# TobiasWooldridge/WaveCap-SDR

Measured on AMD Instinct MI355X. Metric: input IQ MS/s x channels demodulated (1024-channel polyphase filterbank), higher is better.
Workload: dtype f32

## Files before the change

### wavecap-sdr_amd/csrc/pfb.hip

```cpp
#include "pfb_internal.h"
#include "wh_common.h"
#include <cmath>
#include <cstdint>
#include <cstdlib>
#include <memory>
#include <vector>

using namespace wh;

namespace {

constexpr int FM = 1024;
constexpr int FHOP = 512;
constexpr int FT = 9;
constexpr int GH = 4;
constexpr int LDS1_K1 = 272;

template <int FMT>
__device__ __forceinline__ float2 ld_iq(const void *p, long long i) {
    if (FMT == 1) {
        short2 v = reinterpret_cast<const short2 *>(p)[i];
        return make_float2((float)v.x * (1.0f / 32768.0f), (float)v.y * (1.0f / 32768.0f));
    }
    return reinterpret_cast<const float2 *>(p)[i];
}
template <int FMT>
__device__ __forceinline__ float2 ld_iq_raw(const void *p, long long i) {
    if (FMT == 1) {
        short2 v = reinterpret_cast<const short2 *>(p)[i];
        return make_float2((float)v.x, (float)v.y);
    }
    return reinterpret_cast<const float2 *>(p)[i];
}
__device__ __forceinline__ float2 ld_iq_rt(const void *p, int fmt, long long i) {
    return fmt == 1 ? ld_iq<1>(p, i) : ld_iq<0>(p, i);
}

struct PfbFastArgs {
    const void *x;
    float2 *out;
    const float *arms;
    const float2 *tw1024;
    long long first_hop;
    long long n_groups;
    int groups_per_wg;
    int n_wg;
    int alt_dir;
    int map_chunk;
    long long max_block;
    double *stats_ws;
#ifdef WH_DIAG
    int ablate;
#endif
};

typedef float p2f __attribute__((ext_vector_type(2)));
#define P_SW(a) __builtin_shufflevector(a, a, 1, 0)
#define P_XX(a) __builtin_shufflevector(a, a, 0, 0)
#define P_YY(a) __builtin_shufflevector(a, a, 1, 1)
#define P_FMA(a, b, c) __builtin_elementwise_fma(a, b, c)
#define P_PMI(x, d) P_FMA(P_SW(d), (p2f{1.f, -1.f}), x)
#define P_MMI(x, d) P_FMA(P_SW(d), (p2f{-1.f, 1.f}), x)
__device__ __forceinline__ p2f pcmul(p2f a, p2f w) {
    const p2f t = P_XX(a) * w;
    const p2f s = P_YY(a) * p2f{-1.f, 1.f};
    return P_FMA(s, P_SW(w), t);
}
__device__ __forceinline__ p2f pcmulc(p2f a, float wx, float wy) {
    return P_FMA(P_YY(a), (p2f{-wy, wx}), (P_XX(a) * p2f{wx, wy}));
}
__device__ __forceinline__ void pfft4(p2f &a0, p2f &a1, p2f &a2, p2f &a3) {
    const p2f s02 = a0 + a2, d02 = a0 - a2, s13 = a1 + a3, d13 = a1 - a3;
    a0 = s02 + s13;
    a2 = s02 - s13;
    a1 = P_PMI(d02, d13);
    a3 = P_MMI(d02, d13);
}
__device__ __forceinline__ void pfft16(p2f (&v)[16]) {
    constexpr float C1 = 0.92387953251128673848f, S1 = 0.38268343236508978178f, R2 = 0.70710678118654752440f;
#pragma unroll
    for (int na = 0; na < 4; ++na) pfft4(v[na], v[na + 4], v[na + 8], v[na + 12]);
    v[5] = pcmulc(v[5], C1, -S1);
    v[9] = P_PMI(v[9], v[9]) * p2f{R2, R2};
    v[13] = pcmulc(v[13], S1, -C1);
    v[6] = P_PMI(v[6], v[6]) * p2f{R2, R2};
    v[10] = P_SW(v[10]) * p2f{1.f, -1.f};
    v[14] = P_MMI(v[14], v[14]) * p2f{-R2, -R2};
    v[7] = pcmulc(v[7], S1, -C1);
    v[11] = P_MMI(v[11], v[11]) * p2f{-R2, -R2};
    v[15] = pcmulc(v[15], -C1, S1);
#pragma unroll
    for (int kb = 0; kb < 4; ++kb) pfft4(v[4 * kb], v[4 * kb + 1], v[4 * kb + 2], v[4 * kb + 3]);
#pragma unroll
    for (int a = 0; a < 4; ++a)
#pragma unroll
        for (int b = a + 1; b < 4; ++b) {
            const p2f tmp = v[a + 4 * b];
            v[a + 4 * b] = v[b + 4 * a];
            v[b + 4 * a] = tmp;
        }
}

template <int FMT, bool GLDS, bool STATS, bool W3>
struct Pfb1024Lds {
    static constexpr int LDS_HOP = W3 ? 1088 : 1152;
    static constexpr int PRE_BYTES = GLDS ? GH * FHOP * (FMT == 1 ? 4 : 8) : 0;
    static constexpr bool PRE_SINGLE = W3 && FMT == 0;
    static constexpr int WORDS = GH * LDS_HOP + 256 + (PRE_SINGLE ? 1 : 2) * PRE_BYTES / 8;
};

template <int FMT, bool GLDS, bool STATS, bool W3, int DIR>
__device__ __forceinline__ void pfb1024_body(const PfbFastArgs &a, float2 *lds, long long g0, long long g1) {
    constexpr bool ST8 = W3;
    constexpr int LDS2_ROW = W3 ? 17 : 18;
    constexpr int LDS_HOP = Pfb1024Lds<FMT, GLDS, STATS, W3>::LDS_HOP;
    constexpr int PRE_BYTES = Pfb1024Lds<FMT, GLDS, STATS, W3>::PRE_BYTES;
    constexpr bool PRE_SINGLE = Pfb1024Lds<FMT, GLDS, STATS, W3>::PRE_SINGLE;
    float2 *tw256 = lds + GH * LDS_HOP;
    unsigned char *pre0 = reinterpret_cast<unsigned char *>(lds + GH * LDS_HOP + 256);
    constexpr int NEW0 = DIR > 0 ? 9 : 0;

    const int t = threadIdx.x;
    const int lane = t & 63;
    const int wave = t >> 6;

    const float2 tw256_t = a.tw1024[(4 * (t & 15) * (t >> 4)) & 1023];
    float2 tw1 = a.tw1024[t], tw2 = a.tw1024[(2 * t) & 1023], tw3 = a.tw1024[(3 * t) & 1023];
    long long h = a.first_hop + (DIR > 0 ? g0 : g1 - 1) * GH;
    float2 wA[9 + GH], wB[9 + GH];
    const long long xp = (h - 8) * FHOP + t;
#pragma unroll
    for (int i = 0; i < 9 + GH; ++i) {
        wA[i] = ld_iq_raw<FMT>(a.x, xp + i * FHOP);
        wB[i] = ld_iq_raw<FMT>(a.x, xp + i * FHOP + 256);
    }
    typedef float v2f __attribute__((ext_vector_type(2)));
    v2f tpr[(4 * FT) / 2];
#pragma unroll
    for (int e = 0; e < 4 * FT; e += 2) {
        const int q0 = e / FT, j0 = e - q0 * FT, q1 = (e + 1) / FT, j1 = (e + 1) - q1 * FT;
        constexpr float TS = FMT == 1 ? 1.0f / 32768.0f : 1.0f;
        tpr[e / 2] = v2f{a.arms[(t + 256 * q0) * FT + j0] * TS, a.arms[(t + 256 * q1) * FT + j1] * TS};
    }
    tw256[t] = tw256_t;
    __syncthreads();
    const p2f tw1p = {tw1.x, tw1.y}, tw2p = {tw2.x, tw2.y}, tw3p = {tw3.x, tw3.y};
    const p2f tw1r = {-tw1.y, tw1.x}, tw2r = {-tw2.y, tw2.x}, tw3r = {-tw3.y, tw3.x};

    StAcc sacc[STATS ? 4 : 1];
    if (STATS) {
#pragma unroll
        for (int q = 0; q < 4; ++q) stacc_init(sacc[q]);
    }

    constexpr int NJ = GLDS ? PRE_BYTES / 16 / 256 : 0;
    auto dma_copy = [&](unsigned char *dst, long long blk) {
#ifdef WH_DIAG
        if (a.ablate & 2) blk = 9 + (blk & 15);
#endif
        const unsigned char *src = reinterpret_cast<const unsigned char *>(a.x) + (size_t)blk * FHOP * (FMT == 1 ? 4 : 8);
#pragma unroll
        for (int j = 0; j < NJ; ++j) {
            const unsigned char *gp = src + (size_t)(j * 256 + t) * 16;
            unsigned base = (unsigned)(uintptr_t)dst + (unsigned)(j * 256 + wave * 64) * 16;
            base = __builtin_amdgcn_readfirstlane(base);
            unsigned save;
            asm volatile("s_mov_b32 %0, m0\n\t"
                         "s_mov_b32 m0, %1\n\t"
                         "global_load_lds_dwordx4 %2, off\n\t"
                         "s_mov_b32 m0, %0"
                         : "=&s"(save) : "s"(base), "v"(gp) : "memory");
        }
    };
    __builtin_amdgcn_s_waitcnt(0x0F70);
    const long long ng = g1 - g0;
    for (long long it = 0; it < ng; ++it, h += DIR * GH) {
        const bool more = it + 1 < ng;
        unsigned char *pre = pre0 + ((!PRE_SINGLE && (it & 1)) ? PRE_BYTES : 0);
#pragma unroll
        for (int e = 0; e < (4 * FT) / 2; ++e) asm volatile("" : "+v"(tpr[e]));
#define WH_TAP(q, j) ((((q) * FT + (j)) & 1) ? __builtin_shufflevector(tpr[((q) * FT + (j)) >> 1], tpr[((q) * FT + (j)) >> 1], 1, 1) \
                                             : __builtin_shufflevector(tpr[((q) * FT + (j)) >> 1], tpr[((q) * FT + (j)) >> 1], 0, 0))
#define WH_V2(f) (v2f{(f).x, (f).y})
#pragma unroll
        for (int i = 0; i < GH; ++i) {
            v2f p0 = {0.f, 0.f}, p1 = p0, p2 = p0, p3 = p0;
#pragma unroll
            for (int j = 0; j < FT; ++j) {
                p0 = __builtin_elementwise_fma(WH_V2(wA[i + 8 - j]), WH_TAP(0, j), p0);
                p1 = __builtin_elementwise_fma(WH_V2(wB[i + 8 - j]), WH_TAP(1, j), p1);
                p2 = __builtin_elementwise_fma(WH_V2(wA[i + 9 - j]), WH_TAP(2, j), p2);
                p3 = __builtin_elementwise_fma(WH_V2(wB[i + 9 - j]), WH_TAP(3, j), p3);
            }
            pfft4(p0, p1, p2, p3);
            p2f *L = reinterpret_cast<p2f *>(lds + i * LDS_HOP);
            L[t] = p0;
            L[LDS1_K1 + t] = P_FMA(P_YY(p1), tw1r, (P_XX(p1) * tw1p));
            L[2 * LDS1_K1 + t] = P_FMA(P_YY(p2), tw2r, (P_XX(p2) * tw2p));
            L[3 * LDS1_K1 + t] = P_FMA(P_YY(p3), tw3r, (P_XX(p3) * tw3p));
        }
        if (DIR > 0) {
#pragma unroll
            for (int i = 0; i < 9; ++i) {
                wA[i] = wA[i + GH];
                wB[i] = wB[i + GH];
            }
        } else {
#pragma unroll
            for (int i = 8; i >= 0; --i) {
                wA[i + GH] = wA[i];
                wB[i + GH] = wB[i];
            }
        }
        const long long nblk = DIR > 0 ? h + GH + 1 : h - GH - 8;
        auto issue_dma = [&]() {
            if (more) dma_copy(pre, nblk);
        };
        if (GLDS) {
            if (!PRE_SINGLE) issue_dma();
        } else {
#pragma unroll
            for (int i = 0; i < GH; ++i) {
                long long blk = nblk + i;
                blk = blk > a.max_block ? a.max_block : (DIR < 0 && blk < 0 ? 0 : blk);
                wA[NEW0 + i] = ld_iq_raw<FMT>(a.x, blk * FHOP + t);
                wB[NEW0 + i] = ld_iq_raw<FMT>(a.x, blk * FHOP + t + 256);
            }
        }
        __syncthreads();
        if (GLDS && PRE_SINGLE) issue_dma();
        {
            p2f *L = reinterpret_cast<p2f *>(lds + wave * LDS_HOP);
            const int k1 = lane >> 4, n3 = lane & 15;
            p2f v[16];
            {
                const p2f *src = L + k1 * LDS1_K1 + n3;
#pragma unroll
                for (int n2 = 0; n2 < 16; ++n2) v[n2] = src[n2 * 16];
            }
            pfft16(v);
            __builtin_amdgcn_wave_barrier();
            p2f *dst = L + k1 * LDS2_ROW + n3;
            const p2f *twp = reinterpret_cast<const p2f *>(tw256);
            dst[0] = v[0];
#pragma unroll
            for (int k2 = 1; k2 < 16; ++k2) dst[k2 * 4 * LDS2_ROW] = pcmul(v[k2], twp[k2 * 16 + n3]);
        }
        __builtin_amdgcn_wave_barrier();
        {
            float2 *L = lds + wave * LDS_HOP;
            p2f v[16];
            if (W3) {
                const p2f *src = reinterpret_cast<const p2f *>(L) + lane * LDS2_ROW;
#pragma unroll
                for (int j = 0; j < 16; ++j) v[j] = src[j];
            } else {
                typedef float f4 __attribute__((ext_vector_type(4)));
                const unsigned addr = static_cast<unsigned>(reinterpret_cast<uintptr_t>(L + lane * LDS2_ROW));
                f4 r0, r1, r2, r3, r4, r5, r6, r7;
                asm volatile("ds_read_b128 %0, %8\n\t"
                             "ds_read_b128 %1, %8 offset:16\n\t"
                             "ds_read_b128 %2, %8 offset:32\n\t"
                             "ds_read_b128 %3, %8 offset:48\n\t"
                             "ds_read_b128 %4, %8 offset:64\n\t"
                             "ds_read_b128 %5, %8 offset:80\n\t"
                             "ds_read_b128 %6, %8 offset:96\n\t"
                             "ds_read_b128 %7, %8 offset:112\n\t"
                             "s_waitcnt lgkmcnt(0)"
                             : "=&v"(r0), "=&v"(r1), "=&v"(r2), "=&v"(r3), "=&v"(r4), "=&v"(r5), "=&v"(r6), "=&v"(r7)
                             : "v"(addr)
                             : "memory");
                __builtin_amdgcn_sched_barrier(0);
                v[0] = p2f{r0.x, r0.y};   v[1] = p2f{r0.z, r0.w};
                v[2] = p2f{r1.x, r1.y};   v[3] = p2f{r1.z, r1.w};
                v[4] = p2f{r2.x, r2.y};   v[5] = p2f{r2.z, r2.w};
                v[6] = p2f{r3.x, r3.y};   v[7] = p2f{r3.z, r3.w};
                v[8] = p2f{r4.x, r4.y};   v[9] = p2f{r4.z, r4.w};
                v[10] = p2f{r5.x, r5.y};  v[11] = p2f{r5.z, r5.w};
                v[12] = p2f{r6.x, r6.y};  v[13] = p2f{r6.z, r6.w};
                v[14] = p2f{r7.x, r7.y};  v[15] = p2f{r7.z, r7.w};
            }
            pfft16(v);
            float2 vf[16];
#pragma unroll
            for (int j = 0; j < 16; ++j) vf[j] = make_float2(v[j].x, v[j].y);
            if (STATS) {
                float *pwv = reinterpret_cast<float *>(L);
#pragma unroll
                for (int j = 0; j < 16; ++j) pwv[lane + 64 * j] = stat_power(vf[j].x, vf[j].y);
            } else if (ST8) {
                float2 *o = a.out + (h + wave) * FM + lane;
#pragma unroll
                for (int j = 0; j < 16; ++j)
#ifdef WH_DIAG
                    if (!(a.ablate & 1) || vf[j].x == 1.2345e30f)
#endif
                    o[64 * j] = vf[j];
            } else {
                const bool even = (lane & 1) == 0;
                float4 *o4 = reinterpret_cast<float4 *>(a.out + (h + wave) * FM + (lane & ~1) + (even ? 0 : 512));
#pragma unroll
                for (int j = 0; j < 8; ++j) {
                    float2 snd = even ? vf[j + 8] : vf[j];
                    float2 rcv;
                    rcv.x = __shfl_xor(snd.x, 1);
                    rcv.y = __shfl_xor(snd.y, 1);
                    float2 lo = even ? vf[j] : rcv;
                    float2 hi = even ? rcv : vf[j + 8];
#ifdef WH_DIAG
                    if (!(a.ablate & 1) || lo.x == 1.2345e30f)
#endif
                    o4[32 * j] = make_float4(lo.x, lo.y, hi.x, hi.y);
                }
            }
        }
        if (STATS) {
            __syncthreads();
#pragma unroll
            for (int q = 0; q < 4; ++q)
#pragma unroll
                for (int w = 0; w < GH; ++w)
                    stacc_add(sacc[q], reinterpret_cast<const float *>(lds + w * LDS_HOP)[t + 256 * q]);
            if (((it + 1) & 3) == 0) {
#pragma unroll
                for (int q = 0; q < 4; ++q) stacc_fold(sacc[q]);
            }
        }
        if (GLDS) {
#ifdef WH_DIAG
            if (a.ablate) asm volatile("s_waitcnt vmcnt(0)" ::: "memory");
            else
#endif
            if (STATS) asm volatile("s_waitcnt vmcnt(0)" ::: "memory");
            else if (ST8) asm volatile("s_waitcnt vmcnt(16)" ::: "memory");
            else asm volatile("s_waitcnt vmcnt(8)" ::: "memory");
        }
        __syncthreads();
        if (GLDS && more) {
#pragma unroll
            for (int i = 0; i < GH; ++i) {
                if (FMT == 1) {
                    const short2 *p16 = reinterpret_cast<const short2 *>(pre);
                    const short2 va = p16[i * FHOP + t], vb = p16[i * FHOP + t + 256];
                    wA[NEW0 + i] = make_float2((float)va.x, (float)va.y);
                    wB[NEW0 + i] = make_float2((float)vb.x, (float)vb.y);
                } else {
                    const float2 *p32 = reinterpret_cast<const float2 *>(pre);
                    wA[NEW0 + i] = p32[i * FHOP + t];
                    wB[NEW0 + i] = p32[i * FHOP + t + 256];
                }
            }
        }
    }
    if (STATS) {
        double *row = a.stats_ws + (size_t)blockIdx.x * 4 * FM;
#pragma unroll
        for (int q = 0; q < 4; ++q) {
            stacc_fold(sacc[q]);
            const int c = t + 256 * q;
            row[c] = sacc[q].s;
            row[FM + c] = sacc[q].s2;
            row[2 * FM + c] = (double)sacc[q].mn;
            row[3 * FM + c] = (double)sacc[q].mx;
        }
    }
}

template <int FMT, bool GLDS = false, bool STATS = false, bool W3 = false>
__global__ __launch_bounds__(256) __attribute__((amdgpu_waves_per_eu(W3 ? 3 : 2))) void pfb1024_kernel(PfbFastArgs a) {
    __shared__ __attribute__((aligned(16))) float2 lds[Pfb1024Lds<FMT, GLDS, STATS, W3>::WORDS];
    int b = blockIdx.x;
    int nwg = a.n_wg;
    int per = nwg >> 3;
    int run;
    if (a.map_chunk > 0) {
        const int i = b >> 3, ch = i / a.map_chunk;
        run = (ch * 8 + (b & 7)) * a.map_chunk + (i - ch * a.map_chunk);
    } else if (a.map_chunk == -2) {
        run = (nwg & 7) == 0 ? (b & 7) * per + (b >> 3) : b;
    } else {
        run = b;
    }

    long long g0 = (long long)run * a.groups_per_wg;
    long long g1 = g0 + a.groups_per_wg;
    if (g1 > a.n_groups) g1 = a.n_groups;
    if (g0 >= g1) {
        if (STATS) {
            double *row = a.stats_ws + (size_t)blockIdx.x * 4 * FM;
            for (int c = threadIdx.x; c < FM; c += 256) { row[c] = 0.0; row[FM + c] = 0.0; row[2 * FM + c] = INFINITY; row[3 * FM + c] = 0.0; }
        }
        return;
    }

    if (W3 && !STATS && a.alt_dir && (run & 1)) pfb1024_body<FMT, GLDS, STATS, W3, -1>(a, lds, g0, g1);
    else pfb1024_body<FMT, GLDS, STATS, W3, 1>(a, lds, g0, g1);
}

struct PfbGenArgs {
    const void *x;
    int fmt;
    const float2 *hist;
    float2 *out;
    const float *arms;
    const float2 *tw;
    int M, T, log2M;
    int n_radix;
    int radix[16];
    long long hop0;
    long long n_hops;
    long long hop0b;
    long long n_hops_b;
    long long row_b;
};

__device__ __forceinline__ float2 gen_block(const PfbGenArgs &a, long long g, int k) {
    if (g >= 0) return ld_iq_rt(a.x, a.fmt, g * (a.M / 2) + k);
    int col = (int)(-g - 1);
    if (col >= a.T) return make_float2(0.f, 0.f);
    return a.hist[(size_t)k * a.T + col];
}

__global__ __launch_bounds__(256) void pfb_generic_kernel(PfbGenArgs a) {
    extern __shared__ __attribute__((aligned(16))) float2 sm[];
    const long long h = (long long)blockIdx.x < a.n_hops ? a.hop0 + blockIdx.x
                                                          : a.hop0b + ((long long)blockIdx.x - a.n_hops);
    const int M = a.M, T = a.T;
    for (int k = threadIdx.x; k < M; k += blockDim.x) {
        float re = 0.f, im = 0.f;
        for (int j = 0; j < T; ++j) {
            float2 c = gen_block(a, h - j, k);
            float w = a.arms[(size_t)k * T + j];
            re = fmaf(c.x, w, re);
            im = fmaf(c.y, w, im);
        }
        sm[k] = make_float2(re, im);
    }
    __syncthreads();
    const bool in_b = (long long)blockIdx.x >= a.n_hops;
    float2 *o = a.out + (size_t)((in_b && a.row_b >= 0) ? a.row_b + (h - a.hop0b) : h) * M;
    if (a.n_radix > 0) {
        float2 *src = sm, *dst = sm + M;
        int n = M, s = 1;
        for (int st = 0; st < a.n_radix; ++st) {
            const int r = a.radix[st];
            const int m = n / r;
            for (int i = threadIdx.x; i < M / r; i += blockDim.x) {
                const int pp = i / s, q = i - pp * s;
                const float2 *x = src + q + s * pp;
                float2 *y = dst + q + s * r * pp;
                const int sm_ = s * m;
                const int tws = pp * s;
                if (r == 2) {
                    float2 c0 = x[0], c1 = x[sm_];
                    y[0] = cadd(c0, c1);
                    y[s] = cmul(csub(c0, c1), a.tw[tws]);
                } else if (r == 4) {
                    float2 v0 = x[0], v1 = x[sm_], v2 = x[2 * sm_], v3 = x[3 * sm_];
                    fft4(v0, v1, v2, v3);
                    y[0] = v0;
                    y[s] = cmul(v1, a.tw[tws]);
                    y[2 * s] = cmul(v2, a.tw[2 * tws]);
                    y[3 * s] = cmul(v3, a.tw[3 * tws]);
                } else if (r == 3) {
                    const float C = -0.5f, S = -0.86602540378443864676f;
                    float2 v0 = x[0], v1 = x[sm_], v2 = x[2 * sm_];
                    float2 t1 = cadd(v1, v2), t2 = csub(v1, v2);
                    float2 u = make_float2(fmaf(C, t1.x, v0.x), fmaf(C, t1.y, v0.y));
                    float2 w = make_float2(-S * t2.y, S * t2.x);
                    y[0] = cadd(v0, t1);
                    y[s] = cmul(cadd(u, w), a.tw[tws]);
                    y[2 * s] = cmul(csub(u, w), a.tw[2 * tws]);
                } else {
                    const float C1 = 0.30901699437494742410f, S1 = 0.95105651629515357212f;
                    const float C2 = -0.80901699437494742410f, S2 = 0.58778525229247312917f;
                    float2 v0 = x[0], v1 = x[sm_], v2 = x[2 * sm_], v3 = x[3 * sm_], v4 = x[4 * sm_];
                    float2 a1 = cadd(v1, v4), b1 = csub(v1, v4), a2 = cadd(v2, v3), b2 = csub(v2, v3);
                    float2 r1 = make_float2(v0.x + C1 * a1.x + C2 * a2.x, v0.y + C1 * a1.y + C2 * a2.y);
                    float2 r2 = make_float2(v0.x + C2 * a1.x + C1 * a2.x, v0.y + C2 * a1.y + C1 * a2.y);
                    float2 i1 = make_float2(S1 * b1.y + S2 * b2.y, -(S1 * b1.x + S2 * b2.x));
                    float2 i2 = make_float2(S2 * b1.y - S1 * b2.y, -(S2 * b1.x - S1 * b2.x));
                    y[0] = make_float2(v0.x + a1.x + a2.x, v0.y + a1.y + a2.y);
                    y[s] = cmul(cadd(r1, i1), a.tw[tws]);
                    y[2 * s] = cmul(cadd(r2, i2), a.tw[2 * tws]);
                    y[3 * s] = cmul(csub(r2, i2), a.tw[3 * tws]);
                    y[4 * s] = cmul(csub(r1, i1), a.tw[4 * tws]);
                }
            }
            __syncthreads();
            float2 *tmp = src; src = dst; dst = tmp;
            n = m; s *= r;
        }
        for (int k = threadIdx.x; k < M; k += blockDim.x) o[k] = src[k];
    } else if (a.log2M > 0) {
        float2 *src = sm, *dst = sm + M;
        const int half = M >> 1;
        int n = M, s = 1;
        for (int st = 0; st < a.log2M; ++st) {
            const int m = n >> 1;
            for (int i = threadIdx.x; i < half; i += blockDim.x) {
                int pp = i / s, q = i - pp * s;
                float2 c0 = src[q + s * pp];
                float2 c1 = src[q + s * (pp + m)];
                float2 w = a.tw[(size_t)pp * s];
                dst[q + s * 2 * pp] = cadd(c0, c1);
                dst[q + s * (2 * pp + 1)] = cmul(csub(c0, c1), w);
            }
            __syncthreads();
            float2 *tmp = src; src = dst; dst = tmp;
            n = m; s <<= 1;
        }
        for (int k = threadIdx.x; k < M; k += blockDim.x) o[k] = src[k];
    } else {
        for (int c = threadIdx.x; c < M; c += blockDim.x) {
            float re = 0.f, im = 0.f;
            int idx = 0;
            for (int k = 0; k < M; ++k) {
                float2 y = sm[k];
                float2 w = a.tw[idx];
                re += y.x * w.x - y.y * w.y;
                im += y.x * w.y + y.y * w.x;
                idx += c;
                if (idx >= M) idx -= M;
            }
            o[c] = make_float2(re, im);
        }
    }
}

constexpr int RT = 9;
struct PfbRunArgs {
    const void *x;
    float2 *out;
    const float *arms;
    const float2 *tw;
    int M, n_radix;
    int radix[12];
    int stride[12];
    float inv_stride[12];
    long long first_hop, end_hop;
    long long max_block;
    int hops_per_wave;
};

template <int CPL>
__device__ __forceinline__ void run_fft_passes(float2 *img, const float2 *twl, const PfbRunArgs &a, float2 *o,
                                               int lane) {
    const int M = a.M;
    for (int st = 1; st < a.n_radix; ++st) {
// ... 283 lines not shown
    if (sl < slices) {
        const double *p = part + ((size_t)sl * M + c) * 4;
        s = p[0]; s2 = p[1]; mn = p[2]; mx = p[3];
    }
    for (int o = 32; o > 0; o >>= 1) {
        s += __shfl_xor(s, o);
        s2 += __shfl_xor(s2, o);
        mn = fmin(mn, __shfl_xor(mn, o));
        mx = fmax(mx, __shfl_xor(mx, o));
    }
    if (sl != 0) return;
    double *o = stats + (size_t)c * 5;
    if (accumulate && o[2] > 0.0) {
        o[0] += s; o[1] += s2; o[2] += (double)hops;
        o[3] = fmin(o[3], mn); o[4] = fmax(o[4], mx);
    } else {
        o[0] = s; o[1] = s2; o[2] = (double)hops; o[3] = mn; o[4] = mx;
    }
}

__global__ void stats_merge_kernel(const double *g, int R, int M, double *out) {
    const int c = blockIdx.x * blockDim.x + threadIdx.x;
    if (c >= M) return;
    double s0 = 0, s1 = 0, s2 = 0, mn = INFINITY, mx = -INFINITY;
    for (int r = 0; r < R; ++r) {
        const double *p = g + ((size_t)r * M + c) * 5;
        s0 += p[0]; s1 += p[1]; s2 += p[2];
        if (p[2] > 0.0) { mn = fmin(mn, p[3]); mx = fmax(mx, p[4]); }
    }
    double *o = out + (size_t)c * 5;
    o[0] = s0; o[1] = s1; o[2] = s2; o[3] = mn; o[4] = mx;
}

}

struct wh_pfb {
    int M, T, log2M;
    float *d_arms = nullptr;
    float2 *d_tw = nullptr;
    float2 *d_hist[2] = {nullptr, nullptr};
    int cur = 0;
    double *d_part = nullptr;
    float2 *d_sink = nullptr;
    float2 *d_edge = nullptr;
    double *d_stats_ws = nullptr;
    size_t stats_ws_rows = 0;
    int cu_count = 256;
    int gpw_override = 0;
    int map_chunk = 0;
    int alt_dir = 1;
    int ablate = 0;
    int variant = 0;
    int path = 0;
    bool run_ok = false;
    bool mid_ok = false;
    bool prof = false;
    static constexpr int EVR = 64;
    hipEvent_t ev0[EVR] = {}, ev1[EVR] = {};
    int ev_cur = 0, ev_last = -1, ev_n = 0;
    hipStream_t side = nullptr;
    hipEvent_t ev_fork = nullptr, ev_join = nullptr;
    int ev_begin() { ev_cur = (ev_last + 1) % EVR; return ev_cur; }
    void ev_end() { ev_last = ev_cur; if (ev_n < EVR) ++ev_n; }
};

extern "C" int wh_pfb_create(wh_pfb **out, int M, int T, const double *h_arms) {
    if (!out || !h_arms || M < 2 || (M & 1) || T < 1 || T > 64) return set_err(WH_E_ARG, "wh_pfb_create: bad M/T");
    if ((size_t)M * 16 > 160 * 1024) return set_err(WH_E_ARG, "wh_pfb_create: M=%d exceeds the LDS-resident limit", M);
    wh_pfb *p = new wh_pfb();
    std::unique_ptr<wh_pfb, void (*)(wh_pfb *)> guard(p, wh_pfb_destroy);
    p->M = M; p->T = T;
#ifdef WH_DIAG
    if (const char *e = getenv("WH_PFB_ABLATE")) p->ablate = atoi(e);
#endif
    int l2 = 0;
    while ((1 << l2) < M) ++l2;
    p->log2M = ((1 << l2) == M) ? l2 : 0;
    {
        int rem = M;
        while (rem % 2 == 0) rem /= 2;
        while (rem % 3 == 0) rem /= 3;
        while (rem % 5 == 0) rem /= 5;
        p->run_ok = T == RT && M % 4 == 0 && M >= 64 && M <= 512 && M != FM && rem == 1;
    }
    p->mid_ok = pfb_mid_supported(M, T);
    std::vector<float> arms((size_t)M * T);
    for (size_t i = 0; i < arms.size(); ++i) arms[i] = (float)h_arms[i];
    std::vector<float2> tw(M);
    for (int m = 0; m < M; ++m) {
        double ang = -2.0 * M_PI * (double)m / (double)M;
        tw[m] = make_float2((float)cos(ang), (float)sin(ang));
    }
    hipDeviceProp_t prop;
    int dev = 0;
    WH_HIP(hipGetDevice(&dev));
    WH_HIP(hipGetDeviceProperties(&prop, dev));
    p->cu_count = prop.multiProcessorCount;
    if (M == FM && T == FT) {
        if (hipStreamCreateWithFlags(&p->side, hipStreamNonBlocking) != hipSuccess) p->side = nullptr;
        if (p->side && (hipEventCreateWithFlags(&p->ev_fork, hipEventDisableTiming) != hipSuccess ||
                        hipEventCreateWithFlags(&p->ev_join, hipEventDisableTiming) != hipSuccess)) {
            (void)hipStreamDestroy(p->side);
            p->side = nullptr;
        }
    }
    WH_HIP(hipMalloc(&p->d_arms, arms.size() * sizeof(float)));
    WH_HIP(hipMalloc(&p->d_tw, tw.size() * sizeof(float2)));
    WH_HIP(hipMalloc(&p->d_hist[0], (size_t)M * T * sizeof(float2)));
    WH_HIP(hipMalloc(&p->d_hist[1], (size_t)M * T * sizeof(float2)));
    WH_HIP(hipMalloc(&p->d_part, (size_t)64 * M * 4 * sizeof(double)));
    WH_HIP(hipMalloc(&p->d_sink, (size_t)M * sizeof(float2)));
    if (M == FM && T == FT) WH_HIP(hipMalloc(&p->d_edge, (size_t)11 * FM * sizeof(float2)));
    WH_HIP(hipMemcpy(p->d_arms, arms.data(), arms.size() * sizeof(float), hipMemcpyHostToDevice));
    WH_HIP(hipMemcpy(p->d_tw, tw.data(), tw.size() * sizeof(float2), hipMemcpyHostToDevice));
    WH_HIP(hipMemset(p->d_hist[0], 0, (size_t)M * T * sizeof(float2)));
    WH_HIP(hipMemset(p->d_hist[1], 0, (size_t)M * T * sizeof(float2)));
    *out = guard.release();
    return WH_OK;
}

extern "C" void wh_pfb_destroy(wh_pfb *p) {
    if (!p) return;
    (void)hipFree(p->d_arms);
    (void)hipFree(p->d_tw);
    (void)hipFree(p->d_hist[0]);
    (void)hipFree(p->d_hist[1]);
    (void)hipFree(p->d_part);
    (void)hipFree(p->d_sink);
    (void)hipFree(p->d_edge);
    (void)hipFree(p->d_stats_ws);
    for (int i = 0; i < wh_pfb::EVR; ++i) {
        if (p->ev0[i]) (void)hipEventDestroy(p->ev0[i]);
        if (p->ev1[i]) (void)hipEventDestroy(p->ev1[i]);
    }
    if (p->side) {
        (void)hipStreamSynchronize(p->side);
        (void)hipStreamDestroy(p->side);
        (void)hipEventDestroy(p->ev_fork);
        (void)hipEventDestroy(p->ev_join);
    }
    delete p;
}

extern "C" int wh_pfb_tune(wh_pfb *p, int key, int value) {
    if (!p) return set_err(WH_E_ARG, "wh_pfb_tune: null handle");
    switch (key) {
    case WH_PFB_TUNE_PATH:
        if (value < 0 || value > 3) return set_err(WH_E_ARG, "wh_pfb_tune: path %d", value);
        if (value == 2 && !p->run_ok) return set_err(WH_E_ARG, "wh_pfb_tune: the run kernel does not take M=%d T=%d", p->M, p->T);
        if (value == 3 && !p->mid_ok) return set_err(WH_E_ARG, "wh_pfb_tune: no shaped kernel for M=%d T=%d", p->M, p->T);
        p->path = value;
        return WH_OK;
    case WH_PFB_TUNE_PREFETCH:
        if (value != 0 && value != 1 && value != 3 && value != 5 && value != 7 ) return set_err(WH_E_ARG, "wh_pfb_tune: prefetch %d", value);
        p->variant = value;
        return WH_OK;
#ifdef WH_DIAG
    case 4:
        p->ablate = value;
        return WH_OK;
#endif
    case WH_PFB_TUNE_HOPS_PER_RUN:
        if (value < 0 || value > 4096) return set_err(WH_E_ARG, "wh_pfb_tune: hops per run %d", value);
        p->gpw_override = value;
        return WH_OK;
    case WH_PFB_TUNE_RUN_MAP:
        if (value < -2 || value > 4096) return set_err(WH_E_ARG, "wh_pfb_tune: run map %d", value);
        p->map_chunk = value;
        return WH_OK;
    case WH_PFB_TUNE_ALT_DIR:
        if (value != 0 && value != 1) return set_err(WH_E_ARG, "wh_pfb_tune: alt dir %d", value);
        p->alt_dir = value;
        return WH_OK;
    }
    return set_err(WH_E_ARG, "wh_pfb_tune: unknown key %d", key);
}

extern "C" int wh_pfb_profile(wh_pfb *p, int enable) {
    if (!p) return set_err(WH_E_ARG, "wh_pfb_profile: null handle");
    if (enable && !p->ev0[0]) {
        for (int i = 0; i < wh_pfb::EVR; ++i) {
            WH_HIP(hipEventCreate(&p->ev0[i]));
            WH_HIP(hipEventCreate(&p->ev1[i]));
        }
    }
    p->prof = enable != 0;
    p->ev_n = 0;
    p->ev_last = -1;
    return WH_OK;
}

extern "C" int wh_pfb_kernel_ms_back(wh_pfb *p, int back, float *ms) {
    if (!p || !ms) return set_err(WH_E_ARG, "wh_pfb_kernel_ms: null");
    if (back < 0 || back >= p->ev_n) return set_err(WH_E_ARG, "wh_pfb_kernel_ms: no profiled launch %d back (have %d)", back, p->ev_n);
    const int i = ((p->ev_last - back) % wh_pfb::EVR + wh_pfb::EVR) % wh_pfb::EVR;
    WH_HIP(hipEventSynchronize(p->ev1[i]));
    WH_HIP(hipEventElapsedTime(ms, p->ev0[i], p->ev1[i]));
    return WH_OK;
}

extern "C" int wh_pfb_kernel_ms(wh_pfb *p, float *ms) { return wh_pfb_kernel_ms_back(p, 0, ms); }

extern "C" size_t wh_pfb_hops(const wh_pfb *p, size_t n) {
    if (!p || n < (size_t)p->M) return 0;
    return (n - p->M) / (p->M / 2) + 1;
}

static int launch_generic(wh_pfb *p, const void *d_iq, int fmt, float *d_out, long long hop0, long long n_hops,
                          hipStream_t st, long long hop0b = 0, long long n_hops_b = 0, long long row_b = -1) {
    if (n_hops_b < 0) n_hops_b = 0;
    if (n_hops <= 0 && n_hops_b <= 0) return WH_OK;
    if (n_hops < 0) n_hops = 0;
    PfbGenArgs a;
    a.x = d_iq;
    a.fmt = fmt;
    a.hist = p->d_hist[p->cur];
    a.out = reinterpret_cast<float2 *>(d_out);
    a.arms = p->d_arms;
    a.tw = p->d_tw;
    a.M = p->M; a.T = p->T; a.log2M = p->log2M;
    a.hop0 = hop0; a.n_hops = n_hops;
    a.hop0b = hop0b; a.n_hops_b = n_hops_b; a.row_b = row_b;
    a.n_radix = 0;
    {
        int rem = p->M, k = 0;
        int rad[16];
        while (rem % 4 == 0 && k < 16) { rad[k++] = 4; rem /= 4; }
        while (rem % 2 == 0 && k < 16) { rad[k++] = 2; rem /= 2; }
        while (rem % 3 == 0 && k < 16) { rad[k++] = 3; rem /= 3; }
        while (rem % 5 == 0 && k < 16) { rad[k++] = 5; rem /= 5; }
        if (rem == 1 && k > 0) {
            a.n_radix = k;
            for (int i = 0; i < 16; ++i) a.radix[i] = i < k ? rad[i] : 1;
        } else {
            for (int i = 0; i < 16; ++i) a.radix[i] = 1;
        }
    }
    size_t smem = (size_t)p->M * sizeof(float2) * ((p->log2M || a.n_radix) ? 2 : 1);
    if (smem > 64 * 1024) {
        WH_HIP(hipFuncSetAttribute(reinterpret_cast<const void *>(pfb_generic_kernel),
                                   hipFuncAttributeMaxDynamicSharedMemorySize, (int)smem));
    }
    int bt = p->M <= 512 ? 64 : 256;
    if (n_hops + n_hops_b <= 2LL * p->cu_count) bt = 256;
    const long long MAXG = 1 << 30;
    if (n_hops_b > 0) {
        hipLaunchKernelGGL(pfb_generic_kernel, dim3((unsigned)(n_hops + n_hops_b)), dim3(bt), smem, st, a);
        WH_LAUNCH_CHECK();
        return WH_OK;
    }
    for (long long off = 0; off < n_hops; off += MAXG) {
        long long cnt = n_hops - off < MAXG ? n_hops - off : MAXG;
        a.hop0 = hop0 + off;
        a.n_hops = cnt;
        hipLaunchKernelGGL(pfb_generic_kernel, dim3((unsigned)cnt), dim3(bt), smem, st, a);
        WH_LAUNCH_CHECK();
    }
    return WH_OK;
}

static int pfb_run_fmt(wh_pfb *p, const void *d_iq, int fmt, size_t n, float *d_out, void *stream);

extern "C" int wh_pfb_run(wh_pfb *p, const float *d_iq, size_t n, float *d_out, void *stream) {
    return pfb_run_fmt(p, d_iq, 0, n, d_out, stream);
}

extern "C" int wh_pfb_run_i16(wh_pfb *p, const int16_t *d_iq16, size_t n, float *d_out, void *stream) {
    return pfb_run_fmt(p, d_iq16, 1, n, d_out, stream);
}

static int pfb_run_fmt(wh_pfb *p, const void *d_iq, int fmt, size_t n, float *d_out, void *stream) {
    if (!p) return set_err(WH_E_ARG, "wh_pfb_run: null handle");
    hipStream_t st = as_stream(stream);
    long long H = (long long)wh_pfb_hops(p, n);
    if (H == 0) return WH_OK;
    if (!d_iq || !d_out) return set_err(WH_E_ARG, "wh_pfb_run: null buffer");
    int rc;
    const bool fast = (p->M == FM && p->T == FT) && p->path != 1 && !(p->path == 3 && p->mid_ok);
    if (!fast && p->mid_ok && (p->path == 0 || p->path == 3)) {
        PfbMidCall c;
        c.x = d_iq; c.fmt = fmt; c.n = n;
        c.hist = p->d_hist[p->cur]; c.new_hist = p->d_hist[p->cur ^ 1];
        c.out = reinterpret_cast<float2 *>(d_out);
        c.sink = p->d_sink; c.sink_elems = (size_t)p->M;
        c.arms = p->d_arms; c.tw = p->d_tw;
        c.H = H; c.cu_count = p->cu_count; c.hops_per_run = p->gpw_override; c.stats_only = 0;
        c.stats_ws = nullptr; c.stats_out = nullptr; c.stats_accumulate = 0;
#ifdef WH_DIAG
        c.stats_only = p->ablate << 8;
#endif
        if (p->prof) WH_HIP(hipEventRecord(p->ev0[p->ev_begin()], st));
        if ((rc = pfb_mid_launch(p->M, p->T, c, st)) != WH_OK) return rc;
        if (p->prof) {
            WH_HIP(hipEventRecord(p->ev1[p->ev_cur], st));
            p->ev_end();
        }
        p->cur ^= 1;
        return WH_OK;
    }
    const bool run = !fast && p->run_ok && p->path != 1;
    long long head = (fast || run) ? (H < 8 ? H : 8) : H;
    const bool fork = fast && p->side && (H - 8) / GH >= 8LL * p->cu_count;
    hipStream_t sg = st;
    if (fork) {
        WH_HIP(hipEventRecord(p->ev_fork, st));
        WH_HIP(hipStreamWaitEvent(p->side, p->ev_fork, 0));
        sg = p->side;
    }
    {
        long long tail0 = 0, tailn = 0;
        if (fast && H > 8) {
            tail0 = 8 + ((H - 8) / GH) * GH;
            tailn = H - tail0;
        }
        if ((rc = launch_generic(p, d_iq, fmt, d_out, 0, head, sg, tail0, tailn)) != WH_OK) return rc;
    }
    const int hist_nxt = p->cur ^ 1;
    if (fork) {
        hipLaunchKernelGGL(pfb_hist_kernel, dim3((p->M * p->T + 255) / 256), dim3(256), 0, sg, d_iq, fmt, p->d_hist[p->cur],
                           p->d_hist[hist_nxt], p->M, p->T, H);
        WH_LAUNCH_CHECK();
        WH_HIP(hipEventRecord(p->ev_join, sg));
    }
    if (run && H > 8) {
        PfbRunArgs a;
        a.x = d_iq;
        a.out = reinterpret_cast<float2 *>(d_out);
        a.arms = p->d_arms;
        a.tw = p->d_tw;
        a.M = p->M;
        int k = 0, rem = p->M / 4;
        a.radix[k++] = 4;
        while (rem % 4 == 0) { a.radix[k++] = 4; rem /= 4; }
        while (rem % 2 == 0) { a.radix[k++] = 2; rem /= 2; }
        while (rem % 3 == 0) { a.radix[k++] = 3; rem /= 3; }
        while (rem % 5 == 0) { a.radix[k++] = 5; rem /= 5; }
        a.n_radix = k;
        for (int i = 0, s = 1; i < 12; ++i) {
            if (i >= k) a.radix[i] = 1;
            a.stride[i] = s;
            a.inv_stride[i] = 1.0f / (float)s;
            if (i < k) s *= a.radix[i];
        }
        a.first_hop = 8;
        a.end_hop = H;
        a.max_block = (long long)(n / (size_t)(p->M / 2)) - 1;
        const int cpl = p->M <= 256 ? 1 : 2;
        const int rgh = cpl == 1 ? 2 : 1;
        long long nh = H - 8;
        long long hpw = (nh + (long long)p->cu_count * 24 - 1) / ((long long)p->cu_count * 24);
        if (hpw < 8) hpw = 8;
        if (hpw > 64) hpw = 64;
        if (p->gpw_override > 0) hpw = p->gpw_override;
        hpw = (hpw + rgh - 1) / rgh * rgh;
        a.hops_per_wave = (int)hpw;
        const long long waves = (nh + hpw - 1) / hpw;
        const unsigned nwg = (unsigned)((waves + 3) / 4);
        const size_t smem = (size_t)4 * rgh * p->M * sizeof(float2);
        if (p->prof) WH_HIP(hipEventRecord(p->ev0[p->ev_begin()], st));
        if (cpl == 1) {
            if (fmt == 1) hipLaunchKernelGGL((pfb_run_kernel<1, 1, 2>), dim3(nwg), dim3(256), smem, st, a);
            else hipLaunchKernelGGL((pfb_run_kernel<0, 1, 2>), dim3(nwg), dim3(256), smem, st, a);
        } else {
            if (fmt == 1) hipLaunchKernelGGL((pfb_run_kernel<1, 2, 1>), dim3(nwg), dim3(256), smem, st, a);
            else hipLaunchKernelGGL((pfb_run_kernel<0, 2, 1>), dim3(nwg), dim3(256), smem, st, a);
        }
        WH_LAUNCH_CHECK();
        if (p->prof) {
            WH_HIP(hipEventRecord(p->ev1[p->ev_cur], st));
            p->ev_end();
        }
    }
    if (fast && H > 8) {
        long long n_groups = (H - 8) / GH;
        if (n_groups > 0) {
            PfbFastArgs a;
            a.x = d_iq;
            a.out = reinterpret_cast<float2 *>(d_out);
            a.arms = p->d_arms;
            a.tw1024 = p->d_tw;
            a.first_hop = 8;
            a.n_groups = n_groups;
            const bool w3 = p->variant == 0 || p->variant == 5 || p->variant == 7;
            int gpw = w3 ? (fmt == 1 ? 8 : 5) : 64;
            long long nwg = (n_groups + gpw - 1) / gpw;
            while (gpw > 2 && nwg < (long long)p->cu_count * (w3 ? 6 : 8)) {
                gpw = w3 ? gpw - 1 : gpw >> 1;
                nwg = (n_groups + gpw - 1) / gpw;
            }
            if (p->gpw_override > 0) {
                gpw = p->gpw_override;
                nwg = (n_groups + gpw - 1) / gpw;
            }
            a.groups_per_wg = gpw;
            a.n_wg = (int)nwg;
            a.map_chunk = p->map_chunk != 0 ? p->map_chunk : (gpw <= 16 ? 16 : -2);
            a.alt_dir = p->alt_dir;
            if (a.map_chunk > 0) nwg = (nwg + 8LL * a.map_chunk - 1) / (8LL * a.map_chunk) * (8LL * a.map_chunk);
            a.max_block = (long long)(n / (size_t)FHOP) - 1;
#ifdef WH_DIAG
            a.ablate = p->ablate;
#endif
            if (p->prof) WH_HIP(hipEventRecord(p->ev0[p->ev_begin()], st));
            const bool dma = p->variant == 3;
            if (p->variant == 0 || p->variant == 5 || p->variant == 7) {
                if (p->variant != 7) {
                    if (fmt == 1) hipLaunchKernelGGL((pfb1024_kernel<1, true, false, true>), dim3((unsigned)nwg), dim3(256), 0, st, a);
                    else hipLaunchKernelGGL((pfb1024_kernel<0, true, false, true>), dim3((unsigned)nwg), dim3(256), 0, st, a);
                } else {
                    if (fmt == 1) hipLaunchKernelGGL((pfb1024_kernel<1, false, false, true>), dim3((unsigned)nwg), dim3(256), 0, st, a);
                    else hipLaunchKernelGGL((pfb1024_kernel<0, false, false, true>), dim3((unsigned)nwg), dim3(256), 0, st, a);
                }
            } else if (dma) {
                if (fmt == 1) hipLaunchKernelGGL((pfb1024_kernel<1, true>), dim3((unsigned)nwg), dim3(256), 0, st, a);
                else hipLaunchKernelGGL((pfb1024_kernel<0, true>), dim3((unsigned)nwg), dim3(256), 0, st, a);
            } else if (fmt == 1)
                hipLaunchKernelGGL(pfb1024_kernel<1>, dim3((unsigned)nwg), dim3(256), 0, st, a);
            else
                hipLaunchKernelGGL(pfb1024_kernel<0>, dim3((unsigned)nwg), dim3(256), 0, st, a);
            WH_LAUNCH_CHECK();
            if (p->prof) {
                WH_HIP(hipEventRecord(p->ev1[p->ev_cur], st));
                p->ev_end();
            }
        }
    }
    int nxt = hist_nxt;
    if (fork) {
        WH_HIP(hipStreamWaitEvent(st, p->ev_join, 0));
    } else {
        int tot = p->M * p->T;
        hipLaunchKernelGGL(pfb_hist_kernel, dim3((tot + 255) / 256), dim3(256), 0, st, d_iq, fmt, p->d_hist[p->cur],
                           p->d_hist[nxt], p->M, p->T, H);
        WH_LAUNCH_CHECK();
    }
    p->cur = nxt;
    return WH_OK;
}

template <int MODE>
__global__ __launch_bounds__(256) void stream_1r2w_kernel(const float4 *in, float4 *out, size_t n4) {
    const size_t stride = (size_t)gridDim.x * 256 * 4;
    for (size_t i0 = (size_t)blockIdx.x * 256 * 4 + threadIdx.x; i0 < n4; i0 += stride) {
        float4 v[4];
#pragma unroll
        for (int u = 0; u < 4; ++u) v[u] = i0 + u * 256 < n4 ? in[i0 + u * 256] : make_float4(0, 0, 0, 0);
#pragma unroll
        for (int u = 0; u < 4; ++u)
            if (i0 + u * 256 < n4) {
                const size_t i = i0 + u * 256;
                if (MODE == 1) {
                    const size_t o = 2 * (i - threadIdx.x) + threadIdx.x;
                    out[o] = v[u];
                    out[o + 256] = v[u];
                } else if (MODE == 2) {
                    typedef float f4 __attribute__((ext_vector_type(4)));
                    const f4 q = {v[u].x, v[u].y, v[u].z, v[u].w};
                    __builtin_nontemporal_store(q, reinterpret_cast<f4 *>(out + i));
                    __builtin_nontemporal_store(q, reinterpret_cast<f4 *>(out + n4 + i));
                } else {
                    out[i] = v[u];
                    out[n4 + i] = v[u];
                }
            }
    }
}

extern "C" int wh_diag_stream_1r2w(const float *d_in, float *d_out, size_t n, void *stream) {
    if (!d_in || !d_out || (n & 1)) return set_err(WH_E_ARG, "wh_diag_stream_1r2w: null buffer or odd n");
    if (n == 0) return WH_OK;
    const size_t n4 = n / 2;
    size_t blocks = (n4 + 1023) / 1024;
    size_t cap = (size_t)1 << 24;
    int mode = 0;
#ifdef WH_DIAG
    if (const char *e = getenv("WH_DIAG_BLOCKS")) cap = (size_t)atol(e);
    if (const char *e = getenv("WH_DIAG_MODE")) mode = atoi(e);
#endif
    if (blocks > cap) blocks = cap;
    const float4 *in4 = reinterpret_cast<const float4 *>(d_in);
    float4 *out4 = reinterpret_cast<float4 *>(d_out);
    if (mode == 1) hipLaunchKernelGGL(stream_1r2w_kernel<1>, dim3((unsigned)blocks), dim3(256), 0, as_stream(stream), in4, out4, n4);
    else if (mode == 2) hipLaunchKernelGGL(stream_1r2w_kernel<2>, dim3((unsigned)blocks), dim3(256), 0, as_stream(stream), in4, out4, n4);
    else hipLaunchKernelGGL(stream_1r2w_kernel<0>, dim3((unsigned)blocks), dim3(256), 0, as_stream(stream), in4, out4, n4);
    WH_LAUNCH_CHECK();
    return WH_OK;
}

__global__ __launch_bounds__(256) void stream_1r4w_kernel(const float4 *in, float4 *out, size_t n4) {
    const size_t stride = (size_t)gridDim.x * 256 * 4;
    for (size_t i0 = (size_t)blockIdx.x * 256 * 4 + threadIdx.x; i0 < n4; i0 += stride) {
        float4 v[4];
#pragma unroll
        for (int u = 0; u < 4; ++u) v[u] = i0 + u * 256 < n4 ? in[i0 + u * 256] : make_float4(0, 0, 0, 0);
#pragma unroll
        for (int u = 0; u < 4; ++u)
            if (i0 + u * 256 < n4) {
                const size_t i = i0 + u * 256;
                out[i] = v[u];
                out[n4 + i] = v[u];
                out[2 * n4 + i] = v[u];
                out[3 * n4 + i] = v[u];
            }
    }
}

extern "C" int wh_diag_stream_1r4w(const float *d_in, float *d_out, size_t n, void *stream) {
    if (!d_in || !d_out || (n & 1)) return set_err(WH_E_ARG, "wh_diag_stream_1r4w: null buffer or odd n");
    if (n == 0) return WH_OK;
    const size_t n4 = n / 2;
    const size_t blocks = (n4 + 1023) / 1024;
    hipLaunchKernelGGL(stream_1r4w_kernel, dim3((unsigned)blocks), dim3(256), 0, as_stream(stream),
                       reinterpret_cast<const float4 *>(d_in), reinterpret_cast<float4 *>(d_out), n4);
    WH_LAUNCH_CHECK();
    return WH_OK;
}

extern "C" int wh_pfb_run_stats(wh_pfb *p, const void *d_iq, int input_format, size_t n, double *d_stats, int accumulate,
                                void *stream) {
    if (!p) return set_err(WH_E_ARG, "wh_pfb_run_stats: null handle");
    if (input_format != 0 && input_format != 1) return set_err(WH_E_ARG, "wh_pfb_run_stats: input_format 0 (complex64) / 1 (int16)");
    if (!p->mid_ok) return set_err(WH_E_ARG, "wh_pfb_run_stats: no shaped kernel for M=%d T=%d (run + wh_pfb_channel_stats instead)", p->M, p->T);
    hipStream_t st = as_stream(stream);
    const long long H = (long long)wh_pfb_hops(p, n);
    if (H == 0) return WH_OK;
    if (!d_iq || !d_stats) return set_err(WH_E_ARG, "wh_pfb_run_stats: null buffer");
    if (p->M == FM && p->T == FT && p->path != 3 && p->d_edge) {
        int rc;
        const long long n_groups = H > 8 ? (H - 8) / GH : 0;
        const long long head = H < 8 ? H : 8;
        const long long tail0 = 8 + n_groups * GH, tailn = H > 8 ? H - tail0 : 0;
        int acc = accumulate;
        if (n_groups > 0) {
            PfbFastArgs a;
            a.x = d_iq; a.out = nullptr; a.arms = p->d_arms; a.tw1024 = p->d_tw;
            a.first_hop = 8; a.n_groups = n_groups;
            int gpw = 64;
            long long nwg = (n_groups + gpw - 1) / gpw;
            while (gpw > 2 && nwg < (long long)p->cu_count * 8) { gpw >>= 1; nwg = (n_groups + gpw - 1) / gpw; }
            if (nwg > 2LL * p->cu_count) {
                nwg = 2LL * p->cu_count;
                gpw = (int)((n_groups + nwg - 1) / nwg);
                nwg = (n_groups + gpw - 1) / gpw;
            }
            if (p->gpw_override > 0) { gpw = p->gpw_override; nwg = (n_groups + gpw - 1) / gpw; }
            a.groups_per_wg = gpw; a.n_wg = (int)nwg; a.map_chunk = -2; a.alt_dir = 0;
            a.max_block = (long long)(n / (size_t)FHOP) - 1;
#ifdef WH_DIAG
            a.ablate = 0;
#endif
            if ((size_t)nwg > p->stats_ws_rows) {
                WH_HIP(hipStreamSynchronize(st));
                (void)hipFree(p->d_stats_ws);
                p->d_stats_ws = nullptr;
                p->stats_ws_rows = 0;
                WH_HIP(hipMalloc(&p->d_stats_ws, (size_t)nwg * 4 * p->M * sizeof(double)));
                p->stats_ws_rows = (size_t)nwg;
            }
// ... 112 lines not shown
```

Baseline: 220.9 million.

## Use register ring buffer for PFB sample window and packed-FMA complex rotate

```diff
diff --git a/wavecap-sdr_amd/csrc/pfb.hip b/wavecap-sdr_amd/csrc/pfb.hip
--- a/wavecap-sdr_amd/csrc/pfb.hip
+++ b/wavecap-sdr_amd/csrc/pfb.hip
@@ -4,6 +4,7 @@
 #include <cstdint>
 #include <cstdlib>
 #include <memory>
+#include <type_traits>
 #include <vector>
 
 using namespace wh;
@@ -66,6 +67,12 @@
     const p2f s = P_YY(a) * p2f{-1.f, 1.f};
     return P_FMA(s, P_SW(w), t);
 }
+__device__ __forceinline__ p2f pcmul_rot(p2f a, p2f w) {
+    const p2f t = P_XX(a) * w;
+    p2f r;
+    asm("v_pk_fma_f32 %0, %1, %2, %3 op_sel:[1,1,0] op_sel_hi:[1,0,1] neg_lo:[0,1,0]" : "=v"(r) : "v"(a), "v"(w), "v"(t));
+    return r;
+}
 __device__ __forceinline__ p2f pcmulc(p2f a, float wx, float wy) {
     return P_FMA(P_YY(a), (p2f{-wy, wx}), (P_XX(a) * p2f{wx, wy}));
 }
@@ -109,7 +116,7 @@
     static constexpr int WORDS = GH * LDS_HOP + 256 + (PRE_SINGLE ? 1 : 2) * PRE_BYTES / 8;
 };
 
-template <int FMT, bool GLDS, bool STATS, bool W3, int DIR>
+template <int FMT, bool GLDS, bool STATS, bool W3, int DIR, bool RING = false>
 __device__ __forceinline__ void pfb1024_body(const PfbFastArgs &a, float2 *lds, long long g0, long long g1) {
     constexpr bool ST8 = W3;
     constexpr int LDS2_ROW = W3 ? 17 : 18;
@@ -127,7 +134,7 @@
     const float2 tw256_t = a.tw1024[(4 * (t & 15) * (t >> 4)) & 1023];
     float2 tw1 = a.tw1024[t], tw2 = a.tw1024[(2 * t) & 1023], tw3 = a.tw1024[(3 * t) & 1023];
     long long h = a.first_hop + (DIR > 0 ? g0 : g1 - 1) * GH;
-    float2 wA[9 + GH], wB[9 + GH];
+    float2 wA[RING ? 16 : 9 + GH], wB[RING ? 16 : 9 + GH];
     const long long xp = (h - 8) * FHOP + t;
 #pragma unroll
     for (int i = 0; i < 9 + GH; ++i) {
@@ -174,7 +181,10 @@
     };
     __builtin_amdgcn_s_waitcnt(0x0F70);
     const long long ng = g1 - g0;
-    for (long long it = 0; it < ng; ++it, h += DIR * GH) {
+    auto group = [&](long long it, auto PH) {
+        constexpr int P = decltype(PH)::value;
+        auto WI = [](int r) { return RING ? (DIR > 0 ? r + 4 * P : r - 4 * P) & 15 : r; };
+        auto WN = [](int r) { return RING ? (DIR > 0 ? r + 4 * (P + 1) : r - 4 * (P + 1)) & 15 : r; };
         const bool more = it + 1 < ng;
         unsigned char *pre = pre0 + ((!PRE_SINGLE && (it & 1)) ? PRE_BYTES : 0);
 #pragma unroll
@@ -187,19 +197,26 @@
             v2f p0 = {0.f, 0.f}, p1 = p0, p2 = p0, p3 = p0;
 #pragma unroll
             for (int j = 0; j < FT; ++j) {
-                p0 = __builtin_elementwise_fma(WH_V2(wA[i + 8 - j]), WH_TAP(0, j), p0);
-                p1 = __builtin_elementwise_fma(WH_V2(wB[i + 8 - j]), WH_TAP(1, j), p1);
-                p2 = __builtin_elementwise_fma(WH_V2(wA[i + 9 - j]), WH_TAP(2, j), p2);
-                p3 = __builtin_elementwise_fma(WH_V2(wB[i + 9 - j]), WH_TAP(3, j), p3);
+                p0 = __builtin_elementwise_fma(WH_V2(wA[WI(i + 8 - j)]), WH_TAP(0, j), p0);
+                p1 = __builtin_elementwise_fma(WH_V2(wB[WI(i + 8 - j)]), WH_TAP(1, j), p1);
+                p2 = __builtin_elementwise_fma(WH_V2(wA[WI(i + 9 - j)]), WH_TAP(2, j), p2);
+                p3 = __builtin_elementwise_fma(WH_V2(wB[WI(i + 9 - j)]), WH_TAP(3, j), p3);
             }
             pfft4(p0, p1, p2, p3);
             p2f *L = reinterpret_cast<p2f *>(lds + i * LDS_HOP);
             L[t] = p0;
-            L[LDS1_K1 + t] = P_FMA(P_YY(p1), tw1r, (P_XX(p1) * tw1p));
-            L[2 * LDS1_K1 + t] = P_FMA(P_YY(p2), tw2r, (P_XX(p2) * tw2p));
-            L[3 * LDS1_K1 + t] = P_FMA(P_YY(p3), tw3r, (P_XX(p3) * tw3p));
-        }
-        if (DIR > 0) {
+            if (RING) {
+                L[LDS1_K1 + t] = pcmul_rot(p1, tw1p);
+                L[2 * LDS1_K1 + t] = pcmul_rot(p2, tw2p);
+                L[3 * LDS1_K1 + t] = pcmul_rot(p3, tw3p);
+            } else {
+                L[LDS1_K1 + t] = P_FMA(P_YY(p1), tw1r, (P_XX(p1) * tw1p));
+                L[2 * LDS1_K1 + t] = P_FMA(P_YY(p2), tw2r, (P_XX(p2) * tw2p));
+                L[3 * LDS1_K1 + t] = P_FMA(P_YY(p3), tw3r, (P_XX(p3) * tw3p));
+            }
+        }
+        if (RING) {
+        } else if (DIR > 0) {
 #pragma unroll
             for (int i = 0; i < 9; ++i) {
                 wA[i] = wA[i + GH];
@@ -223,8 +240,8 @@
             for (int i = 0; i < GH; ++i) {
                 long long blk = nblk + i;
                 blk = blk > a.max_block ? a.max_block : (DIR < 0 && blk < 0 ? 0 : blk);
-                wA[NEW0 + i] = ld_iq_raw<FMT>(a.x, blk * FHOP + t);
-                wB[NEW0 + i] = ld_iq_raw<FMT>(a.x, blk * FHOP + t + 256);
+                wA[WN(NEW0 + i)] = ld_iq_raw<FMT>(a.x, blk * FHOP + t);
+                wB[WN(NEW0 + i)] = ld_iq_raw<FMT>(a.x, blk * FHOP + t + 256);
             }
         }
         __syncthreads();
@@ -244,7 +261,8 @@
             const p2f *twp = reinterpret_cast<const p2f *>(tw256);
             dst[0] = v[0];
 #pragma unroll
-            for (int k2 = 1; k2 < 16; ++k2) dst[k2 * 4 * LDS2_ROW] = pcmul(v[k2], twp[k2 * 16 + n3]);
+            for (int k2 = 1; k2 < 16; ++k2)
+                dst[k2 * 4 * LDS2_ROW] = RING ? pcmul_rot(v[k2], twp[k2 * 16 + n3]) : pcmul(v[k2], twp[k2 * 16 + n3]);
         }
         __builtin_amdgcn_wave_barrier();
         {
@@ -342,15 +360,33 @@
                 if (FMT == 1) {
                     const short2 *p16 = reinterpret_cast<const short2 *>(pre);
                     const short2 va = p16[i * FHOP + t], vb = p16[i * FHOP + t + 256];
-                    wA[NEW0 + i] = make_float2((float)va.x, (float)va.y);
-                    wB[NEW0 + i] = make_float2((float)vb.x, (float)vb.y);
+                    wA[WN(NEW0 + i)] = make_float2((float)va.x, (float)va.y);
+                    wB[WN(NEW0 + i)] = make_float2((float)vb.x, (float)vb.y);
                 } else {
                     const float2 *p32 = reinterpret_cast<const float2 *>(pre);
-                    wA[NEW0 + i] = p32[i * FHOP + t];
-                    wB[NEW0 + i] = p32[i * FHOP + t + 256];
+                    wA[WN(NEW0 + i)] = p32[i * FHOP + t];
+                    wB[WN(NEW0 + i)] = p32[i * FHOP + t + 256];
                 }
             }
         }
+    };
+    if (RING) {
+        for (long long it = 0;;) {
+            group(it, std::integral_constant<int, 0>{});
+            h += DIR * GH;
+            if (++it == ng) break;
+            group(it, std::integral_constant<int, 1>{});
+            h += DIR * GH;
+            if (++it == ng) break;
+            group(it, std::integral_constant<int, 2>{});
+            h += DIR * GH;
+            if (++it == ng) break;
+            group(it, std::integral_constant<int, 3>{});
+            h += DIR * GH;
+            if (++it == ng) break;
+        }
+    } else {
+        for (long long it = 0; it < ng; ++it, h += DIR * GH) group(it, std::integral_constant<int, 0>{});
     }
     if (STATS) {
         double *row = a.stats_ws + (size_t)blockIdx.x * 4 * FM;
@@ -366,7 +402,7 @@
     }
 }
 
-template <int FMT, bool GLDS = false, bool STATS = false, bool W3 = false>
+template <int FMT, bool GLDS = false, bool STATS = false, bool W3 = false, bool RING = false>
 __global__ __launch_bounds__(256) __attribute__((amdgpu_waves_per_eu(W3 ? 3 : 2))) void pfb1024_kernel(PfbFastArgs a) {
     __shared__ __attribute__((aligned(16))) float2 lds[Pfb1024Lds<FMT, GLDS, STATS, W3>::WORDS];
     int b = blockIdx.x;
@@ -393,8 +429,8 @@
         return;
     }
 
-    if (W3 && !STATS && a.alt_dir && (run & 1)) pfb1024_body<FMT, GLDS, STATS, W3, -1>(a, lds, g0, g1);
-    else pfb1024_body<FMT, GLDS, STATS, W3, 1>(a, lds, g0, g1);
+    if (W3 && !STATS && a.alt_dir && (run & 1)) pfb1024_body<FMT, GLDS, STATS, W3, -1, RING>(a, lds, g0, g1);
+    else pfb1024_body<FMT, GLDS, STATS, W3, 1, RING>(a, lds, g0, g1);
 }
 
 struct PfbGenArgs {
@@ -984,7 +1020,7 @@
         p->path = value;
         return WH_OK;
     case WH_PFB_TUNE_PREFETCH:
-        if (value != 0 && value != 1 && value != 3 && value != 5 && value != 7 ) return set_err(WH_E_ARG, "wh_pfb_tune: prefetch %d", value);
+        if (value != 0 && value != 1 && value != 3 && value != 5 && value != 7 && value != 9) return set_err(WH_E_ARG, "wh_pfb_tune: prefetch %d", value);
         p->variant = value;
         return WH_OK;
 #ifdef WH_DIAG
@@ -1213,7 +1249,7 @@
             a.tw1024 = p->d_tw;
             a.first_hop = 8;
             a.n_groups = n_groups;
-            const bool w3 = p->variant == 0 || p->variant == 5 || p->variant == 7;
+            const bool w3 = p->variant == 0 || p->variant == 5 || p->variant == 7 || p->variant == 9;
             int gpw = w3 ? (fmt == 1 ? 8 : 5) : 64;
             long long nwg = (n_groups + gpw - 1) / gpw;
             while (gpw > 2 && nwg < (long long)p->cu_count * (w3 ? 6 : 8)) {
@@ -1235,7 +1271,10 @@
 #endif
             if (p->prof) WH_HIP(hipEventRecord(p->ev0[p->ev_begin()], st));
             const bool dma = p->variant == 3;
-            if (p->variant == 0 || p->variant == 5 || p->variant == 7) {
+            if (p->variant == 0 || p->variant == 9) {
+                if (fmt == 1) hipLaunchKernelGGL((pfb1024_kernel<1, true, false, true, true>), dim3((unsigned)nwg), dim3(256), 0, st, a);
+                else hipLaunchKernelGGL((pfb1024_kernel<0, true, false, true, true>), dim3((unsigned)nwg), dim3(256), 0, st, a);
+            } else if (p->variant == 5 || p->variant == 7) {
                 if (p->variant != 7) {
                     if (fmt == 1) hipLaunchKernelGGL((pfb1024_kernel<1, true, false, true>), dim3((unsigned)nwg), dim3(256), 0, st, a);
                     else hipLaunchKernelGGL((pfb1024_kernel<0, true, false, true>), dim3((unsigned)nwg), dim3(256), 0, st, a);
```

After: 222.2 million (median of 6 runs). Within noise of the previous version (+0.6%).
